# powturbo/Turbo-Range-Coder

Measured on AMD Instinct MI355X. Metric: encode+decode MB/s, order-0 static-CDF rANS, 100 MB bytes, higher is better.
Workload: dtype u32; 1 GPU; text100m: 100000000 B/GPU, static-CDF rANS, 2 states (anscdf4senc/anscdf4sdec per chunk), tables in LDS, chunk 512 B, 1 lane = 1 chunk, 64 chunks/wave; codec=anscdf4s, chunk=512, bytes_per_gpu=100000000, compressed_bytes_per_gpu=64522350, steps_in_flight=1, exchange=none

## Files before the change

include/trc_hip.h:

```cpp
#ifndef TRC_HIP_H_
#define TRC_HIP_H_
#include <stddef.h>
#include <stdint.h>

#ifdef __cplusplus
extern "C" {
#endif

enum trc_codec {
    TRC_ANS4S = 1,
    TRC_RCS1  = 2,
    TRC_RCS2  = 3,
    TRC_RCA   = 4,
    TRC_ANSA  = 5,
    TRC_RCB   = 6,
    TRC_RCAI  = 7,
    TRC_RCA4  = 8,
    TRC_RCAI4 = 9,
    TRC_ANSA4 = 10,
    TRC_RCSM  = 11,
    TRC_ANSO1 = 12,
    TRC_ANSB  = 13,
    TRC_VLCU16 = 14,  TRC_VLCU32 = 15,
    TRC_VLCV16 = 16,  TRC_VLCV32 = 17,
// ... 289 lines not shown
                               uint8_t *filters_out, trc_planes_advice *advice );
size_t trc_planes_advise_batch_work_bytes(const trc_planes_item *items, size_t count, unsigned esize, uint32_t chunk);
int    trc_planes_advise_batch_dev(unsigned filters, const trc_planes_item *items, size_t count, unsigned esize, uint32_t chunk,
                                   uint8_t *filters_out, trc_planes_advice *advice,
                                   void *d_work, size_t work_bytes, void *stream);

#define TRC_PLANES_BATCH_MAGIC 0x42435254u
typedef struct trc_planes_batch_hdr {
    uint32_t magic;
    uint8_t  version;
    uint8_t  esize;
    uint16_t zero;
    uint32_t chunk;
    uint32_t zero2;
    uint64_t count;
    uint64_t inner;
    uint64_t size;
    uint64_t bytes;
} trc_planes_batch_hdr;
typedef struct trc_planes_batch_layout {
    uint64_t inner;
    uint64_t off[8];
    uint64_t size;
} trc_planes_batch_layout;
enum { TRC_ITEMS_HOST = 0, TRC_ITEMS_DEV = 1 };
uint32_t trc_planes_batch_auto_chunk(int codec, const trc_planes_item *items, size_t count, unsigned esize);
size_t trc_planes_batch_bound(int codec, const trc_planes_item *items, size_t count, unsigned esize, uint32_t chunk, unsigned cdfnum);
int    trc_planes_batch_layout_host(int codec, const trc_planes_item *items, size_t count, unsigned esize, uint32_t chunk,
                                    unsigned cdfnum, const uint64_t *total, trc_planes_batch_layout *L);
int    trc_planes_batch_check(const void *buf, size_t buflen, size_t count_expected);
int    trc_planes_batch_info(const void *buf, size_t buflen, trc_planes_batch_hdr *h, uint64_t *n, uint8_t *filters, size_t cap);
int trc_planes_batch_pack_dev(int codec, const trc_planes_item *items, const uint8_t *filters, size_t count,
                              unsigned esize, uint32_t chunk, const uint16_t *d_cdf, unsigned cdfnum,
                              const int32_t *d_status, const uint32_t *d_clen, const void *d_payload,
                              const uint64_t *d_total, void *d_out, size_t out_bytes, uint64_t *d_size, void *stream);
int trc_decode_planes_batch_packed_dev(int codec, const void *d_cont, size_t cont_bytes,
                                       const trc_planes_item *items, const uint8_t *filters, size_t count, size_t first_item, size_t item_count,
                                       unsigned esize, uint32_t chunk, unsigned cdfnum, const uint64_t *total ,
                                       void *d_work, size_t work_bytes, void *stream);
size_t trc_encode_planes_batch_host(int codec, const trc_planes_item *items, const uint8_t *filters ,
                                    size_t count, unsigned esize, uint32_t chunk, unsigned cdfnum, int items_on,
                                    void *out, size_t outcap);
size_t trc_encode_aplanes_batch_host(int codec, const trc_planes_item *items, size_t count, unsigned esize, uint32_t chunk,
                                     unsigned cdfnum, int items_on, void *out, size_t outcap, uint8_t *filters_out );
size_t trc_decode_planes_batch_host(const void *in, size_t inlen, const trc_planes_item *items, size_t count,
                                    size_t first_item, size_t item_count, int items_on);

int trc_timing_enable(int on);
int trc_timing_pause(int paused);
int trc_timing_read(int decode, double *total_ms, int *launches);

const char *trc_kernel_name(int codec, int decode);

#ifdef __cplusplus
}
#endif
#endif
```

turbo-range-coder_amd/csrc/trc_api.hip:

```cpp
#include <hip/hip_runtime.h>
#include <mutex>
#include <stdarg.h>
#include <stdio.h>
#include <stdlib.h>
#include <string.h>

#include "../../include/trc_hip.h"
#include "trc_launch.h"

typedef unsigned short cdf_t;
static const unsigned TRC_PROB_ONE_HOST = 32768u;

static thread_local char g_err[512];
static int fail(int code, const char *fmt, ...)
{
    va_list ap; va_start(ap, fmt);
    vsnprintf(g_err, sizeof g_err, fmt, ap);
    va_end(ap);
    fprintf(stderr, "turborc_hip: ERROR: %s\n", g_err);
    return code;
}
int trc_fail(int code, const char *fmt, ...)
{
    va_list ap; va_start(ap, fmt);
// ... 117 lines not shown
#undef NONE
static constexpr int TRC_NCODECS = (int)(sizeof g_codecs / sizeof g_codecs[0]);
static constexpr bool rows_in_id_order()
{
    for (int i = 0; i < TRC_NCODECS; i++) if (g_codecs[i].id != i) return false;
    return true;
}
static_assert(rows_in_id_order(), "g_codecs[i] must be the row of id i");
static const TrcCodec &codec_row(int codec) { return g_codecs[codec > 0 && codec < TRC_NCODECS ? codec : 0]; }
static bool codec_ok(int codec) { return codec_row(codec).enc != nullptr; }
static bool ss_prm_ok(unsigned v) { return !(v & ~0x0f0fu) && (v & 0x0fu) && (v & 0x0f00u); }

static uint32_t g_chunk = 0;
static bool chunk_ok(uint32_t c) { return c >= TRC_CHUNK_MIN && c <= TRC_CHUNK_MAX && (c % 64u) == 0; }
extern "C" uint32_t trc_auto_chunk_codec(int codec, size_t n)
{
    static const uint32_t ladder[] = { 16384u, 12288u, 8192u, 6144u, 4096u, 3072u, 2048u, 1536u, 1024u, 768u, 512u };
    const TrcCodec &r = codec_row(codec);
    const double link_ns = 0.35 * (double)n / 50.0;
    const double budget_ns = link_ns > 1.7e6 ? link_ns : 1.7e6;
    const uint32_t lo = r.floor ? r.floor : TRC_CHUNK_AUTO_MIN;
    for (uint32_t c : ladder)
        if (c <= r.auto_max && (c <= lo || (double)r.wave_ns * c <= budget_ns)) return c;
    return lo;
}
extern "C" uint32_t trc_auto_chunk(size_t n) { return trc_auto_chunk_codec(TRC_ANS4S, n); }
#define TRC_ROUND_CHUNK_MAX 16384u
extern "C" uint32_t trc_round_chunk(int codec, size_t n)
{
    const TrcCodec &r = codec_row(codec);
    if (r.floor) return r.floor;
    const size_t rc = r.round_lanes;
    const size_t cap = r.chunk_max < TRC_ROUND_CHUNK_MAX ? r.chunk_max : TRC_ROUND_CHUNK_MAX;
    for (size_t k = 1;; k++) {
        size_t c = (n + rc * k - 1) / (rc * k);
        c = (c + 63u) & ~(size_t)63u;
        if (c <= cap) return c < TRC_CHUNK_AUTO_MIN ? TRC_CHUNK_AUTO_MIN : (uint32_t)c;
    }
}
extern "C" uint32_t trc_get_chunk(void)
{
    if (!g_chunk) {
        const char *e = getenv("TRC_CHUNK");
        uint32_t c = e ? (uint32_t)strtoul(e, 0, 10) : 0;
        g_chunk = chunk_ok(c) ? c : ~0u;
    }
    return g_chunk == ~0u ? 0u : g_chunk;
}
extern "C" int trc_set_chunk(uint32_t chunk)
{
    if (chunk == 0) { g_chunk = ~0u; return TRC_OK; }
    if (!chunk_ok(chunk)) return fail(TRC_E_ARG, "chunk %u: must be 0 (automatic) or a multiple of 64 in [%u,%u]", chunk, TRC_CHUNK_MIN, TRC_CHUNK_MAX);
    g_chunk = chunk;
    return TRC_OK;
}

#define TRC_INKERNEL_SCAN_MAX 8192u
static inline size_t up256(size_t x) { return (x + 255) & ~(size_t)255; }
static inline size_t scratch2_bytes(const TrcCodec &r, size_t nchunks, uint32_t chunk)
{
    const size_t rows = r.s2_lanes ? ((nchunks + 63) & ~(size_t)63) : nchunks;
    return up256(rows * ((size_t)r.s2_mul * chunk + r.s2_add) + 256);
}
static inline size_t model_area_bytes(const TrcCodec &r, size_t nchunks) { return r.model_area ? up256(r.model_area(r, nchunks)) : 0; }

extern "C" size_t trc_work_bytes(int codec, size_t n, uint32_t chunk)
{
    if (!codec) return 4096;
    const TrcCodec &r = codec_row(codec);
    if (!r.enc || !chunk_ok(chunk)) return 0;
    const size_t nchunks = (n + chunk - 1) / chunk, ngroups = (nchunks + 63) / 64;
    return up256(TRC_TAB_BYTES) + up256(4 * ngroups) + up256(8 * (ngroups + 1)) +
           up256(nchunks * ((size_t)chunk + r.pad)) + scratch2_bytes(r, nchunks, chunk) + model_area_bytes(r, nchunks) +
           (r.aux ? up256(nchunks * 8) : 0) + 4096;
}

static int carve(const TrcCodec &r, size_t n, uint32_t chunk, void *d_work, size_t work_bytes, TrcWork &w)
{
    const size_t need = trc_work_bytes(r.id, n, chunk);
    if (!need || work_bytes < need) return fail(TRC_E_WORK, "workspace %zu B < required %zu B", work_bytes, need);
    if (((uintptr_t)d_work) & 255) return fail(TRC_E_ARG, "workspace must be 256-byte aligned");
    const size_t nchunks = (n + chunk - 1) / chunk, ngroups = (nchunks + 63) / 64;
    uint8_t *p = (uint8_t *)d_work;
    w.tables = p;               p += up256(TRC_TAB_BYTES);
    w.gsum = (uint32_t *)p;     p += up256(4 * ngroups);
    static const uint32_t scan_max = getenv("TRC_SCAN_MAX") ? (uint32_t)atoi(getenv("TRC_SCAN_MAX")) : TRC_INKERNEL_SCAN_MAX;
    w.goff_area = (uint64_t *)p;
    w.goff = ngroups > scan_max ? (uint64_t *)p : nullptr;     p += up256(8 * (ngroups + 1));
    w.scratch = p;
    w.stride = chunk + r.pad;
    w.stride2 = r.s2_mul * chunk + r.s2_add;
    w.scratch2 = p + up256(nchunks * (size_t)w.stride);
    w.model = w.scratch2 + scratch2_bytes(r, nchunks, chunk);
    w.aux = (uint32_t *)(w.model + model_area_bytes(r, nchunks));
    w.nchunks = (uint32_t)nchunks; w.ngroups = (uint32_t)ngroups;
    return TRC_OK;
}

static int check_common(int codec, size_t n, uint32_t chunk, const uint16_t *d_cdf, unsigned cdfnum)
{
    const TrcCodec &r = codec_row(codec);
    if (!r.enc) return fail(TRC_E_ARG, "codec %d not available", codec);
    if (!chunk_ok(chunk)) return fail(TRC_E_ARG, "chunk %u: must be a multiple of 64 in [%u,%u]", chunk, TRC_CHUNK_MIN, TRC_CHUNK_MAX);
    if ((n + chunk - 1) / chunk > 0x7fffffffu) return fail(TRC_E_ARG, "too many chunks");
    if (chunk > r.chunk_max) return fail(TRC_E_ARG, "codec %d: chunk %u exceeds %u", r.id, chunk, r.chunk_max);
    if (r.cdf && (!d_cdf || cdfnum < 1 || cdfnum > 256)) return fail(TRC_E_CDF, "static coder needs a CDF with 1..256 symbols");
// ... 493 lines not shown
```

turbo-range-coder_amd/csrc/trc_dev.h:

```cpp
#pragma once
#include <hip/hip_runtime.h>
#include <stdint.h>

typedef uint8_t  u8;
typedef uint16_t u16;
typedef uint32_t u32;
typedef uint64_t u64;

#define TRC_WAVE        64
#define TRC_PROB_BITS   15u
#define TRC_PROB_ONE    (1u << TRC_PROB_BITS)
#define TRC_ANS_LOW     (1u << 15)

typedef u32 u32_a1 __attribute__((aligned(1)));
typedef u32 u32_a2 __attribute__((aligned(2)));
struct __attribute__((packed, aligned(2))) trc_u128_a2 { u32 x, y, z, w; };

__device__ __forceinline__ uint4 trc_ld16_a2(const u8 *p)
{
    trc_u128_a2 v = *(const trc_u128_a2 *)p;
    return make_uint4(v.x, v.y, v.z, v.w);
}
__device__ __forceinline__ u32 trc_ld32_a2(const u8 *p) { return *(const u32_a2 *)p; }

// ... 138 lines not shown
        for (u32 i = lane; i < len; i += 64) dst[i] = src[i];
        return;
    }
    u32 head = (u32)((16u - ((uintptr_t)dst & 15u)) & 15u);
    if (head > len) head = len;
    if (lane < head) dst[lane] = src[lane];
    const u32 nvec = (len - head) >> 4;
    u8 *d = dst + head; const u8 *s = src + head;
    for (u32 i = lane; i < nvec; i += 64)
        *(uint4 *)(d + (size_t)i * 16) = trc_ld16_a2(s + (size_t)i * 16);
    const u32 done = head + (nvec << 4);
    if (lane < len - done) dst[done + lane] = src[done + lane];
}

__device__ __forceinline__ void trc_wave_copy_raw(u64 rawmask, u64 off, u32 len, u8 *out_wave, u32 chunk, const u8 *payload)
{
    const u32 lane = trc_lane(), grp = lane >> 4, gl = lane & 15u;
    if (((uintptr_t)out_wave | chunk) & 15u) {
        while (rawmask) {
            const int k = __ffsll((long long)rawmask) - 1;
            rawmask &= rawmask - 1;
            const u32 olo = (u32)__shfl((int)(u32)off, k, 64), ohi = (u32)__shfl((int)(u32)(off >> 32), k, 64);
            const u32 l = (u32)__shfl((int)len, k, 64);
            trc_wave_copy(out_wave + (u64)(u32)k * chunk, payload + (((u64)ohi << 32) | olo), l);
        }
        return;
    }
    while (rawmask) {
        int mine = -1;
#pragma unroll
        for (u32 g = 0; g < 4; g++) {
            const int k = rawmask ? __ffsll((long long)rawmask) - 1 : -1;
            if (rawmask) rawmask &= rawmask - 1;
            if (g == grp) mine = k;
        }
        const int src_lane = mine < 0 ? 0 : mine;
        const u32 olo = (u32)__shfl((int)(u32)off, src_lane, 64), ohi = (u32)__shfl((int)(u32)(off >> 32), src_lane, 64);
        const u32 l = (u32)__shfl((int)len, src_lane, 64);
        if (mine >= 0) {
            u8 *d = out_wave + (u64)(u32)mine * chunk;
            const u8 *sp = payload + (((u64)ohi << 32) | olo);
            const u32 nvec = l >> 4;
            for (u32 i = gl; i < nvec; i += 16) *(uint4 *)(d + (size_t)i * 16) = trc_ld16_a2(sp + (size_t)i * 16);
            const u32 done = nvec << 4;
            if (gl < l - done) d[done + gl] = sp[done + gl];
        }
    }
}

__device__ __forceinline__ u64 trc_group_base(const u64 *goff, const u32 *gsum, u32 g)
{
    if (goff) return goff[g];
    u64 acc = 0;
    u32 i = trc_lane();
    for (; i + 448u < g; i += 512u) {
        const u32 a0 = gsum[i], a1 = gsum[i + 64], a2 = gsum[i + 128], a3 = gsum[i + 192];
        const u32 a4 = gsum[i + 256], a5 = gsum[i + 320], a6 = gsum[i + 384], a7 = gsum[i + 448];
        acc += (u64)a0 + a1 + a2 + a3 + ((u64)a4 + a5 + a6 + a7);
    }
    for (; i < g; i += 64) acc += gsum[i];
    u32 lo = (u32)acc, hi = (u32)(acc >> 32);
#pragma unroll
    for (int d = 32; d >= 1; d >>= 1) {
        const u32 l2 = (u32)__shfl_xor((int)lo, d, 64), h2 = (u32)__shfl_xor((int)hi, d, 64);
        const u64 t = ((((u64)hi) << 32) | lo) + ((((u64)h2) << 32) | l2);
        lo = (u32)t; hi = (u32)(t >> 32);
    }
    return (((u64)hi) << 32) | lo;
}

__device__ __forceinline__ float trc_u2f(u32 v)
{
    float r;
    asm("v_cvt_f32_u32_e32 %0, %1" : "=v"(r) : "v"(v));
    return r;
}

__device__ __forceinline__ u32 trc_rans_step(u32 st, u32 f, u32 g, u32 c0)
{
    const u32 q = (u32)((float)st * __builtin_amdgcn_rcpf((float)f));
    const int rm = (int)(st - __umul24(q, f));
    const u32 qe = q + (u32)(rm >> 31) + (rm >= (int)f ? 1u : 0u);
    return st + __umul24(qe, g) + c0;
}
```

turbo-range-coder_amd/csrc/trc_dir.hip:

```cpp
#include <stdlib.h>
#include "trc_dev.h"
#include "trc_launch.h"

__global__ __launch_bounds__(256) void trc_static_prep_kernel(const u16 *__restrict__ cdf, u32 cdfnum,
                                                              u8 *__restrict__ tables)
{
    __shared__ u32 c[258];
    const u32 tid = threadIdx.x;
    for (u32 i = tid; i < 258; i += 256) c[i] = (i <= cdfnum) ? (u32)cdf[i] : TRC_PROB_ONE;
    __syncthreads();
    const u32 slot = blockIdx.x * 256 + tid;
    u32 x = 0, hi = 256;
    while (x + 1 < hi) { u32 mid = (x + hi) >> 1; if (c[mid] > slot) hi = mid; else x = mid; }
    tables[TRC_TAB_LUT + slot] = (u8)x;
    if (blockIdx.x == 0) {
        const u32 c0 = c[tid], f = c[tid + 1] - c0;
        uint4 e; u32 d;
        if (f == 0) {
            e = make_uint4(0u, 0u, 0xffffffffu, 0u); d = 1u << 16;
        } else if (f == 1) {
            e = make_uint4(0xffffffffu, TRC_PROB_ONE - 1u, 1u << 16, c0 + TRC_PROB_ONE - 1u); d = (1u << 16) | c0;
        } else {
            const u32 l = 32u - (u32)__clz((int)(f - 1));
            const u32 m = (u32)((((u64)1) << (31 + l)) / f) + 1u;
// ... 43 lines not shown
        for (u32 k = 0; k < wid; k++) wbase += wsum[k];
        const u64 base = base_s;
        if (i < ngroups) goff[i] = base + wbase + inc - v;
        __syncthreads();
        if (tid == 1023) base_s = base + wbase + inc;
        __syncthreads();
    }
    if (tid == 0) { goff[ngroups] = base_s; if (total) *total = base_s; }
}
void trc_launch_scan_groups(const uint32_t *gsum, uint32_t ngroups, uint64_t *goff, uint64_t *d_total, hipStream_t s)
{
    TRC_LAUNCH_TIMED(trc_scan_groups_kernel, dim3(1), dim3(1024), 0, s, gsum, ngroups, goff, d_total);
}

__global__ __launch_bounds__(256) void trc_range_dir_kernel(const u32 *__restrict__ clen, u32 nchunks, u64 n, u32 chunk,
                                                            const u64 *__restrict__ goff_full, u32 first, u32 count,
                                                            u32 *__restrict__ gsum_sub, u64 *__restrict__ goff_sub)
{
    const u32 ngroups_sub = (count + 63u) >> 6, end = first + count;
    const u32 j = blockIdx.x * 4u + (threadIdx.x >> 6), lane = trc_lane();
    if (j > ngroups_sub) return;
    const u32 b = trc_min(first + 64u * j, end);
    auto clamped = [&](u32 c) -> u32 {
        const u64 left = n - (u64)c * chunk;
        return trc_min(clen[c], left < chunk ? (u32)left : chunk);
    };
    const u32 below = (b & ~63u) + lane, mine = b + lane;
    const u32 pre = trc_wave_sum(below < b ? clamped(below) : 0u);
    const u32 sum = trc_wave_sum(mine < end ? clamped(mine) : 0u);
    if (lane == 0) {
        goff_sub[j] = goff_full[b >> 6] + pre;
        if (j < ngroups_sub) gsum_sub[j] = sum;
    }
}
void trc_launch_range_dir(const uint32_t *d_clen, uint32_t nchunks, size_t n, uint32_t chunk, const uint64_t *goff_full,
                          uint32_t first, uint32_t count, uint32_t *gsum_sub, uint64_t *goff_sub, hipStream_t s)
{
    const uint32_t waves = (count + 63u) / 64u + 1u;
    hipLaunchKernelGGL(trc_range_dir_kernel, dim3((waves + 3u) / 4u), dim3(256), 0, s, d_clen, nchunks, (u64)n, chunk, goff_full,
                       first, count, gsum_sub, goff_sub);
}

#ifndef TRC_GATHER_VPT
#define TRC_GATHER_VPT 6
#endif
#ifndef TRC_GATHER_ATTR
#define TRC_GATHER_ATTR
#endif
template <int PARTS>
__global__ __launch_bounds__(256) TRC_GATHER_ATTR void trc_gather_kernel(const u8 *__restrict__ in, u64 n, u32 chunk, u32 nchunks,
                                                         const u8 *__restrict__ scratch, u32 stride, int from_end,
                                                         const u8 *__restrict__ scratch2, u32 stride2, const u32 *__restrict__ aux,
                                                         const u32 *__restrict__ clen, const u64 *__restrict__ goff,
                                                         const u32 *__restrict__ gsum, u32 ngroups,
                                                         u8 *__restrict__ payload, u64 *__restrict__ total, u64 *__restrict__ goff_out)
{
    constexpr u32 NP = 64u * PARTS;
    constexpr u32 TPP = 256u / NP;
    constexpr u32 VPT = TRC_GATHER_VPT;
    __shared__ u32 ex_s[NP + 1];
    __shared__ u64 src_s[NP];
    __shared__ u64 base_s;
    const u32 g = blockIdx.x, tid = threadIdx.x, lane = tid & 63u, wid = tid >> 6;
    if (wid == 1 || blockDim.x == 64) {
        const u64 b = trc_group_base(goff, gsum, g);
        if (lane == 0) { base_s = b; if (goff_out) goff_out[g] = b; }
    }
    if (wid == 0) {
        const u32 c = g * 64 + lane;
        const u32 l = c < nchunks ? clen[c] : 0u;
        const u64 cstart = (u64)c * chunk;
        const u32 len = c < nchunks ? (u32)((n - cstart) < chunk ? (n - cstart) : chunk) : 0u;
        const bool raw = l == len;
        const u32 inc = trc_wave_incl_scan(l);
        if (PARTS == 1) {
            ex_s[lane] = inc - l;
            src_s[lane] = (u64)(uintptr_t)(raw ? in + cstart : from_end ? scratch + (u64)(c + 1) * stride - l : scratch + (u64)c * stride);
        } else {
            const u8 *a = scratch + (u64)c * stride;
            const u32 la = (raw || c >= nchunks) ? l : from_end >= 3 ? aux[2 * c] : 4u + *(const u32 *)a;
            ex_s[2 * lane] = inc - l; ex_s[2 * lane + 1] = inc - l + la;
            src_s[2 * lane] = (u64)(uintptr_t)(raw ? in + cstart : from_end == 4 ? scratch + (u64)(c + 1) * stride - la : a);
            src_s[2 * lane + 1] = (u64)(uintptr_t)(from_end == 3 ? scratch + (u64)(c + 1) * stride - (l - la) :
                                                   from_end == 4 ? scratch2 + (u64)(c + 1) * stride2 - (l - la) : scratch2 + (u64)c * stride2);
        }
        if (lane == 63) ex_s[NP] = inc;
    }
    __syncthreads();
    const u64 base = base_s;
    const u32 tot = ex_s[NP];
    if (total && g == ngroups - 1 && tid == 0) *total = base + tot;
    u8 *dst0 = payload + base;
    auto src_of = [&](u32 p) -> const u8 * { return (const u8 *)(uintptr_t)src_s[p]; };

    u32 head = (u32)((16u - ((uintptr_t)dst0 & 15u)) & 15u);
    if (head > tot) head = tot;
    const u32 nvec = (tot - head) >> 4;
    const u32 tail0 = head + (nvec << 4);
    for (u32 b = tid; b < head + (tot - tail0); b += 256) {
        const u32 d = b < head ? b : tail0 + (b - head);
        u32 lo = 0, hi = NP;
        while (lo + 1 < hi) { const u32 mid = (lo + hi) >> 1; if (ex_s[mid] <= d) lo = mid; else hi = mid; }
        dst0[d] = src_of(lo)[d - ex_s[lo]];
    }
    {
        const u32 k = tid / TPP, sub = tid % TPP;
        const u32 e0 = ex_s[k], e1 = ex_s[k + 1];
        const u32 v_lo = e0 <= head ? 0u : (e0 - head + 15u) >> 4;
        u32 v_hi = e1 <= head ? 0u : (e1 - head + 15u) >> 4;
        if (v_hi > nvec) v_hi = nvec;
        const u8 *sa = src_of(k);
        const u8 *sb = k + 1 < NP ? src_of(k + 1) : sa;
        const u32 e2 = ex_s[k + 2 > NP ? NP : k + 2];
        const u32 pl = e1 - e0;
        const bool a16 = pl >= 16u;
        const bool b16 = k + 1 < NP && e2 - e1 >= 16u;
        auto bytewise = [&](u32 dv) {
            u32 kk = k;
            const u8 *p = sa;
            for (u32 q = 0; q < 16; q++) {
                while (dv + q >= ex_s[kk + 1]) { kk++; p = src_of(kk); }
                dst0[dv + q] = p[dv + q - ex_s[kk]];
            }
        };
        if (!a16) {
            if (sub == 0 && v_lo < v_hi) bytewise(head + (v_lo << 4));
            return;
        }
        for (u32 v0 = v_lo + sub; v0 < v_hi; v0 += VPT * TPP) {
            uint4 a[VPT], b[VPT];
            u32 d[VPT];
            bool ok[VPT];
#pragma unroll
            for (int j = 0; j < (int)VPT; j++) {
                const u32 v = v0 + TPP * (u32)j;
                ok[j] = v < v_hi;
                d[j] = head + ((ok[j] ? v : v0) << 4);
                a[j] = make_uint4(0u, 0u, 0u, 0u);
                if (ok[j]) a[j] = trc_ld16_a2_global(sa + trc_min(d[j] - e0, pl - 16u));
                b[j] = a[j];
            }
#pragma unroll
            for (int j = 0; j < (int)VPT; j++)
                if (ok[j] && d[j] + 16u > e1 && b16) b[j] = trc_ld16_a2_global(sb);
#pragma unroll
            for (int j = 0; j < (int)VPT; j++) {
                if (!ok[j]) continue;
                const u32 sp = e1 - d[j];
                if (sp >= 16u) { *(uint4 *)(dst0 + d[j]) = a[j]; continue; }
                if (b16) *(uint4 *)(dst0 + d[j]) = trc_splice16(a[j], b[j], 16u - sp);
                else bytewise(d[j]);
            }
        }
    }
}
void trc_launch_gather(const uint8_t *d_in, size_t n, uint32_t chunk, const TrcWork &w, TrcGather mode,
                       const uint32_t *d_clen, uint8_t *d_payload, uint64_t *d_total, hipStream_t s)
{
    const int from_end = mode;
    if (from_end >= 2)
        TRC_LAUNCH_TIMED((trc_gather_kernel<2>), dim3(w.ngroups), dim3(256), 0, s, d_in, (u64)n, chunk, w.nchunks,
                           w.scratch, w.stride, from_end >= 3 ? from_end : 0, w.scratch2, w.stride2, w.aux, d_clen, w.goff, w.gsum, w.ngroups,
                           d_payload, w.goff ? (u64 *)nullptr : d_total, w.goff ? (u64 *)nullptr : w.goff_area);
    else
        TRC_LAUNCH_TIMED((trc_gather_kernel<1>), dim3(w.ngroups), dim3(256), 0, s, d_in, (u64)n, chunk, w.nchunks,
                           w.scratch, w.stride, from_end, w.scratch2, w.stride2, w.aux, d_clen, w.goff, w.gsum, w.ngroups,
                           d_payload, w.goff ? (u64 *)nullptr : d_total, w.goff ? (u64 *)nullptr : w.goff_area);
}

#define TRC_HIST2_WAVE_LDS (128u * 16u * 4u)
#define TRC_HIST2_WAVES 16u
#define TRC_HIST2_ROUND_VECS 1023u
__global__ __launch_bounds__(1024) void trc_hist2_kernel(const u8 *__restrict__ in, u64 n, u64 *__restrict__ hist, u32 round_vecs)
{
    extern __shared__ __attribute__((aligned(16))) u8 smem[];
    typedef __attribute__((address_space(3))) u32 lds_u32;
    const u32 tid = threadIdx.x, lane = tid & 63u, wv = tid >> 6;
    u32 *mine = (u32 *)(smem + wv * TRC_HIST2_WAVE_LDS);
    u64 *tot = (u64 *)(smem + TRC_HIST2_WAVES * TRC_HIST2_WAVE_LDS);
    const u32 col = trc_lds_addr(mine) + (lane & 15u) * 4u;
    if (tid < 256u) tot[tid] = 0;
    const u64 nvec = n >> 4, stride = (u64)gridDim.x * 1024;
    const uint4 *v = (const uint4 *)in;
    auto count = [&](u32 w) __attribute__((always_inline)) {
#pragma unroll
        for (int k = 0; k < 4; k++) {
            const u32 a = (__builtin_amdgcn_ubfe(w, 8 * k + 1, 7) << 6) + col;
            const u32 inc = __umul24(__builtin_amdgcn_ubfe(w, 8 * k, 1), 0xffffu) + 1u;
            __hip_atomic_fetch_add((lds_u32 *)(uintptr_t)a, inc, __ATOMIC_RELAXED, __HIP_MEMORY_SCOPE_WAVEFRONT);
        }
    };
    auto count4 = [&](const uint4 q) __attribute__((always_inline)) { count(q.x); count(q.y); count(q.z); count(q.w); };
    for (u64 r0 = 0; r0 == 0 || r0 < nvec; r0 += stride * round_vecs) {
        for (u32 r = lane; r < 128u * 16u; r += 64u) mine[r] = 0;
        u64 i = r0 + (u64)blockIdx.x * 1024 + tid;
        u32 left = round_vecs;
        if (left >= 2u && i + stride < nvec) {
            uint4 q0 = v[i], q1 = v[i + stride];
            left -= 2u; i += 2 * stride;
            for (; left >= 2u && i + stride < nvec; left -= 2u, i += 2 * stride) {
                const uint4 n0 = v[i], n1 = v[i + stride];
                count4(q0); count4(q1);
                q0 = n0; q1 = n1;
            }
            count4(q0); count4(q1);
        }
        for (; left && i < nvec; left--, i += stride) count4(v[i]);
        if (r0 == 0 && blockIdx.x == 0 && wv == 0)
            for (u64 t = (nvec << 4) + lane; t < n; t += 64) {
                const u32 b = in[t];
                __hip_atomic_fetch_add((lds_u32 *)(uintptr_t)(col + (b >> 1) * 64u), (b & 1u) ? 0x10000u : 1u, __ATOMIC_RELAXED, __HIP_MEMORY_SCOPE_WAVEFRONT);
            }
        u32 lo0 = 0, hi0 = 0, lo1 = 0, hi1 = 0;
#pragma unroll
        for (u32 c4 = 0; c4 < 4u; c4++) {
            const uint4 a = *(const uint4 *)(mine + lane * 16u + c4 * 4u), b = *(const uint4 *)(mine + (lane + 64u) * 16u + c4 * 4u);
            lo0 += (a.x & 0xffffu) + (a.y & 0xffffu) + (a.z & 0xffffu) + (a.w & 0xffffu); hi0 += (a.x >> 16) + (a.y >> 16) + (a.z >> 16) + (a.w >> 16);
            lo1 += (b.x & 0xffffu) + (b.y & 0xffffu) + (b.z & 0xffffu) + (b.w & 0xffffu); hi1 += (b.x >> 16) + (b.y >> 16) + (b.z >> 16) + (b.w >> 16);
        }
// ... 60 lines not shown
```

turbo-range-coder_amd/csrc/trc_launch.h:

```cpp
#pragma once
#include <hip/hip_runtime.h>
#include <hip/hip_ext.h>
#include <stddef.h>
#include <stdint.h>
#include <stdlib.h>

bool trc_tm_next(hipEvent_t *start, hipEvent_t *stop);
#define TRC_LAUNCH_TIMED(kern, grid, block, lds, stream, ...)                                                      \
    do {                                                                                                         \
        hipEvent_t tm_a_, tm_b_;                                                                                 \
        if (trc_tm_next(&tm_a_, &tm_b_)) hipExtLaunchKernelGGL(kern, grid, block, (uint32_t)(lds), stream, tm_a_, tm_b_, 0, __VA_ARGS__); \
        else hipLaunchKernelGGL(kern, grid, block, lds, stream, __VA_ARGS__);                                    \
    } while (0)

bool trc_first_use_on_device(unsigned long long *mask);
#define TRC_RAISE_LDS_ONCE(kern, bytes)                                                                            \
    do {                                                                                                         \
        static unsigned long long seen_ = 0;                                                                     \
        if (trc_first_use_on_device(&seen_))                                                                     \
            (void)hipFuncSetAttribute((const void *)kern, hipFuncAttributeMaxDynamicSharedMemorySize, (int)(bytes)); \
    } while (0)

#define TRC_LDS_ONE_PER_CU (82u * 1024u)
static inline bool trc_nib_big(uint32_t ngroups)
{
    static const int env = getenv("TRC_NIB_BIG") ? atoi(getenv("TRC_NIB_BIG")) : -1;
    return env >= 0 ? env != 0 : (ngroups >= 2048u && ngroups <= 12u * 256u);
}

struct TrcGate { const uint32_t *flag; uint32_t part; };
extern thread_local TrcGate trc_gate_tls;
struct TrcProg { uint32_t *counters; uint32_t *host_flags; uint32_t part; };
extern thread_local TrcProg trc_prog_tls;
bool trc_prog_ok(int codec);
bool trc_gate_ok(int codec);

struct TrcWork {
    uint8_t  *tables;
    uint32_t *gsum;
    uint64_t *goff;
    uint64_t *goff_area;
    uint8_t  *scratch;
    uint32_t  stride;
    uint8_t  *scratch2;
    uint32_t  stride2;
    uint32_t  nchunks, ngroups;
    uint8_t  *model;
    uint32_t *aux;
    uint32_t  ss_prm;
};
#define TRC_O1_MODEL_BYTES (256u * 17u * 32u)

#define TRC_TAB_ENC   0
#define TRC_TAB_DEC   4096
#define TRC_TAB_LUT   8192
#define TRC_TAB_CDF   40960
#define TRC_TAB_BYTES 45056

void trc_launch_static_prep(const uint16_t *d_cdf, unsigned cdfnum, uint8_t *tables, hipStream_t s);

enum TrcGather {
    TRC_GATHER_START = 0,
    TRC_GATHER_END = 1,
    TRC_GATHER_TWO = 2,
    TRC_GATHER_AUX = 3,
    TRC_GATHER_VLA = 4,
};

void trc_launch_group_sums(const uint32_t *d_clen, uint32_t nchunks, size_t n, uint32_t chunk, uint32_t *gsum, hipStream_t s);
void trc_launch_scan_groups(const uint32_t *gsum, uint32_t ngroups, uint64_t *goff, uint64_t *d_total, hipStream_t s);
void trc_launch_range_dir(const uint32_t *d_clen, uint32_t nchunks, size_t n, uint32_t chunk, const uint64_t *goff_full,
                          uint32_t first, uint32_t count, uint32_t *gsum_sub, uint64_t *goff_sub, hipStream_t s);
void trc_launch_gather(const uint8_t *d_in, size_t n, uint32_t chunk, const TrcWork &w, TrcGather mode,
                       const uint32_t *d_clen, uint8_t *d_payload, uint64_t *d_total, hipStream_t s);

struct TrcCodec;
typedef void TrcEncFn(const TrcCodec &c, const uint8_t *d_in, size_t n, uint32_t chunk, const TrcWork &w, uint32_t *d_clen, hipStream_t s);
typedef void TrcDecFn(const TrcCodec &c, const uint8_t *d_payload, const uint32_t *d_clen, size_t n, uint32_t chunk,
                      const TrcWork &w, uint8_t *d_out, hipStream_t s);

struct TrcCodec {
    int id;
    TrcEncFn *enc;
    TrcDecFn *dec;
    int8_t k;
    int8_t streams;
    int8_t nibble;
    bool low4;
    int8_t variant;
    int8_t zz;
    int8_t elem;
    TrcGather gather;
    bool cdf;
    bool ss;
    bool aux;
    bool gate;
    bool prog;
    uint16_t wave_ns;
    uint32_t round_lanes;
    uint32_t auto_max;
    uint32_t floor;
    uint32_t chunk_max;
    uint16_t pad;
    uint8_t s2_mul;
    uint16_t s2_add;
    bool s2_lanes;
    size_t (*model_area)(const TrcCodec &c, size_t nchunks);
    size_t (*slice_model)(const TrcCodec &c);
    const char *kernel_enc, *kernel_dec;
};

TrcEncFn trc_launch_ans4s_enc;  TrcDecFn trc_launch_ans4s_dec;
TrcEncFn trc_launch_rcs_enc;    TrcDecFn trc_launch_rcs_dec;
TrcEncFn trc_launch_rcb_enc;    TrcDecFn trc_launch_rcb_dec;
TrcEncFn trc_launch_o1bit_enc;  TrcDecFn trc_launch_o1bit_dec;
TrcEncFn trc_launch_int_enc;    TrcDecFn trc_launch_int_dec;
size_t trc_int_model_bytes(int k, size_t ngroups);
TrcEncFn trc_launch_bvlc_enc;   TrcDecFn trc_launch_bvlc_dec;
size_t trc_bvlc_model_bytes(int k, size_t nchunks);
TrcEncFn trc_launch_word_enc;   TrcDecFn trc_launch_word_dec;
size_t trc_word_model_bytes(int k);
size_t trc_word_slots(int k, size_t nchunks);
TrcEncFn trc_launch_nibbit_enc; TrcDecFn trc_launch_nibbit_dec;
TrcEncFn trc_launch_ssbit_enc;  TrcDecFn trc_launch_ssbit_dec;
void trc_o1bit_fill(uint8_t *model, size_t bytes, hipStream_t s);
TrcEncFn trc_launch_rca_enc;    TrcDecFn trc_launch_rca_dec;
TrcEncFn trc_launch_rcv_enc;    TrcDecFn trc_launch_rcv_dec;
// ... 13 lines not shown
```

turbo-range-coder_amd/trc.py:

```python
import ctypes as C
import os
import subprocess

import numpy as np

PKG = os.path.dirname(os.path.abspath(__file__))
ROOT = os.path.dirname(PKG)
LIB = os.environ.get("TRC_LIB") or os.path.join(PKG, "libturborc_hip.so")

ANS4S, RCS1, RCS2, RCA, ANSA, RCB, RCAI, RCA4, RCAI4, ANSA4, RCSM, ANSO1, ANSB = 1, 2, 3, 4, 5, 6, 7, 8, 9, 10, 11, 12, 13
VLCU16, VLCU32, VLCV16, VLCV32, VLCVZ16, VLCVZ32 = 14, 15, 16, 17, 18, 19
VLAU16, VLAUZ16, VLAV16, VLAVZ16, VLAV32, VLAVZ32 = 20, 21, 22, 23, 24, 25
RCV8, RCVI8 = 26, 27
RCC1, RCX1 = 28, 29
RCG8, RCG16, RCG32, RCGZ8, RCGZ16, RCGZ32 = 30, 31, 32, 33, 34, 35
RCR8, RCR16, RCR32, RCRZ8, RCRZ16, RCRZ32 = 36, 37, 38, 39, 40, 41
INTBIT = ((RCG8, 1), (RCG16, 2), (RCG32, 4), (RCGZ8, 1), (RCGZ16, 2), (RCGZ32, 4),
          (RCR8, 1), (RCR16, 2), (RCR32, 4), (RCRZ8, 1), (RCRZ16, 2), (RCRZ32, 4))
RCBV16, RCBV32, RCBVZ16, RCBVZ32, RCBVG16, RCBVG32, RCBVGZ16, RCBVGZ32 = 43, 44, 45, 46, 47, 48, 49, 50
BVLC = ((RCBV16, 2), (RCBV32, 4), (RCBVZ16, 2), (RCBVZ32, 4),
        (RCBVG16, 2), (RCBVG32, 4), (RCBVGZ16, 2), (RCBVGZ32, 4))
RCW16, RCW32, RCCW32, RCC2W32 = 52, 53, 54, 55
WORD = ((RCW16, 2), (RCW32, 4), (RCCW32, 4), (RCC2W32, 4))
RC4, RC4C, RCU3 = 58, 59, 60
# ... 165 lines not shown
        l.trc_encode_planes_batch_dev.restype = C.c_int
        l.trc_encode_planes_batch_dev.argtypes = [C.c_int, _it, _sz, C.c_uint, C.c_uint32, _vp, C.c_uint, _vp, _vp, _vp, _vp, _vp, _sz, _vp]
        l.trc_decode_planes_batch_dev.restype = C.c_int
        l.trc_decode_planes_batch_dev.argtypes = [C.c_int, _vp, _vp, _it, _sz, _sz, _sz, C.c_uint, C.c_uint32, _vp, C.c_uint, _vp, _sz, _vp]
        _fl = C.POINTER(C.c_uint8)
        l.trc_planes_split_fbatch_dev.restype = C.c_int
        l.trc_planes_split_fbatch_dev.argtypes = [_it, _fl] + l.trc_planes_split_batch_dev.argtypes[1:]
        l.trc_planes_join_fbatch_dev.restype = C.c_int
        l.trc_planes_join_fbatch_dev.argtypes = [_vp, _sz, _it, _fl] + l.trc_planes_join_batch_dev.argtypes[3:]
        l.trc_encode_fplanes_batch_dev.restype = C.c_int
        l.trc_encode_fplanes_batch_dev.argtypes = [C.c_int, _it, _fl] + l.trc_encode_planes_batch_dev.argtypes[2:]
        l.trc_decode_fplanes_batch_dev.restype = C.c_int
        l.trc_decode_fplanes_batch_dev.argtypes = [C.c_int, _vp, _vp, _it, _fl] + l.trc_decode_planes_batch_dev.argtypes[4:]
        _ad = C.POINTER(PlanesAdvice)
        l.trc_planes_hist_batch_bytes.restype = _sz; l.trc_planes_hist_batch_bytes.argtypes = [_sz, C.c_uint]
        l.trc_planes_hist_batch_dev.restype = C.c_int
        l.trc_planes_hist_batch_dev.argtypes = [C.c_uint, _it, _sz, _sz, _sz, C.c_uint, C.c_uint32, _vp, _vp, _sz, _vp]
        l.trc_planes_advise_batch.restype = C.c_int
        l.trc_planes_advise_batch.argtypes = [_vp, C.c_uint, C.c_uint, _it, _sz, _fl, _ad]
        l.trc_planes_advise_batch_work_bytes.restype = _sz; l.trc_planes_advise_batch_work_bytes.argtypes = [_it, _sz, C.c_uint, C.c_uint32]
        l.trc_planes_advise_batch_dev.restype = C.c_int
        l.trc_planes_advise_batch_dev.argtypes = [C.c_uint, _it, _sz, C.c_uint, C.c_uint32, _fl, _ad, _vp, _sz, _vp]
        l.trc_planes_batch_auto_chunk.restype = C.c_uint32; l.trc_planes_batch_auto_chunk.argtypes = [C.c_int, _it, _sz, C.c_uint]
        l.trc_planes_batch_bound.restype = _sz; l.trc_planes_batch_bound.argtypes = [C.c_int, _it, _sz, C.c_uint, C.c_uint32, C.c_uint]
        l.trc_planes_batch_layout_host.restype = C.c_int
        l.trc_planes_batch_layout_host.argtypes = [C.c_int, _it, _sz, C.c_uint, C.c_uint32, C.c_uint, C.POINTER(C.c_uint64), C.POINTER(PlanesBatchLayout)]
        l.trc_planes_batch_check.restype = C.c_int; l.trc_planes_batch_check.argtypes = [_vp, _sz, _sz]
        l.trc_planes_batch_info.restype = C.c_int
        l.trc_planes_batch_info.argtypes = [_vp, _sz, C.POINTER(PlanesBatchHdr), C.POINTER(C.c_uint64), _fl, _sz]
        l.trc_planes_batch_pack_dev.restype = C.c_int
        l.trc_planes_batch_pack_dev.argtypes = [C.c_int, _it, _fl, _sz, C.c_uint, C.c_uint32, _vp, C.c_uint, _vp, _vp, _vp, _vp, _vp, _sz, _vp, _vp]
        l.trc_decode_planes_batch_packed_dev.restype = C.c_int
        l.trc_decode_planes_batch_packed_dev.argtypes = [C.c_int, _vp, _sz, _it, _fl, _sz, _sz, _sz, C.c_uint, C.c_uint32, C.c_uint,
                                                         C.POINTER(C.c_uint64), _vp, _sz, _vp]
        l.trc_encode_planes_batch_host.restype = _sz
        l.trc_encode_planes_batch_host.argtypes = [C.c_int, _it, _fl, _sz, C.c_uint, C.c_uint32, C.c_uint, C.c_int, _vp, _sz]
        l.trc_encode_aplanes_batch_host.restype = _sz
        l.trc_encode_aplanes_batch_host.argtypes = [C.c_int, _it, _sz, C.c_uint, C.c_uint32, C.c_uint, C.c_int, _vp, _sz, _fl]
        l.trc_decode_planes_batch_host.restype = _sz
        l.trc_decode_planes_batch_host.argtypes = [_vp, _sz, _it, _sz, _sz, _sz, C.c_int]
        l.trc_encode_host.restype = _sz; l.trc_encode_host.argtypes = [C.c_int, _vp, _sz, C.c_uint32, _vp, _sz, _vp, C.c_uint]
        l.trc_decode_host.restype = _sz; l.trc_decode_host.argtypes = [C.c_int, _vp, _sz, _vp, _sz, _vp, C.c_uint]
        l.trc_container_bound.restype = _sz; l.trc_container_bound.argtypes = [_sz, C.c_uint32]
        l.trc_container_check.restype = C.c_int; l.trc_container_check.argtypes = [_vp, _sz, C.c_int, _sz]
        l.trc_host_plan.restype = C.c_int
        l.trc_host_plan.argtypes = [C.c_int, _sz, C.c_uint32, C.c_int, C.c_int, C.POINTER(_sz), C.c_int, C.POINTER(C.c_uint32)]
        l.trc_host_pin.restype = C.c_int; l.trc_host_pin.argtypes = [_vp, _sz]
        l.trc_host_unpin.restype = C.c_int; l.trc_host_unpin.argtypes = [_vp]
        l.trc_timing_enable.restype = C.c_int; l.trc_timing_enable.argtypes = [C.c_int]
        l.trc_timing_pause.restype = C.c_int; l.trc_timing_pause.argtypes = [C.c_int]
        l.trc_timing_read.restype = C.c_int
        l.trc_timing_read.argtypes = [C.c_int, C.POINTER(C.c_double), C.POINTER(C.c_int)]
        l.trc_kernel_name.restype = C.c_char_p; l.trc_kernel_name.argtypes = [C.c_int, C.c_int]
        l.trc_set_devices.restype = C.c_int; l.trc_set_devices.argtypes = [C.POINTER(C.c_int), C.c_int]
        l.trc_get_devices.restype = C.c_int; l.trc_get_devices.argtypes = [C.POINTER(C.c_int), C.c_int]
        _lib = l
    return _lib


class TrcError(RuntimeError):
    pass


def _chk(rc):
    if rc != 0:
        raise TrcError("libturborc_hip rc=%d: %s" % (rc, lib().trc_last_error().decode()))


def timing_enable(on=True):
    _chk(lib().trc_timing_enable(1 if on else 0))


def timing_pause(paused=True):
    _chk(lib().trc_timing_pause(1 if paused else 0))


def timing_read(decode):
    ms, cnt = C.c_double(0), C.c_int(0)
    _chk(lib().trc_timing_read(2 if decode == 2 else 1 if decode else 0, C.byref(ms), C.byref(cnt)))
    return ms.value, cnt.value


def ss_prm(prm):
    return int(prm[0]) | int(prm[1]) << 8


def _cdfnum(codec, cdfnum, prm):
    return cdfnum if codec in STATIC else ss_prm(prm) if codec in SSBIT else 0


def nchunks(n, chunk):
    return (n + chunk - 1) // chunk


def range_work_bytes(codec, n, chunk, count):
    return lib().trc_range_work_bytes(codec, n, chunk, count)


class DeviceCoder:

    def __init__(self, codec, n, chunk=4096, device="cuda"):
        import torch
        self.torch = torch
        self.codec, self.n, self.chunk = codec, n, chunk
        self.nch = nchunks(n, chunk)
        self.dev = torch.device(device)
        u8 = torch.uint8
        self.work_bytes = lib().trc_work_bytes(codec, n, chunk)
        if self.work_bytes == 0:
            raise TrcError("bad (codec, n, chunk)")
        self.work = torch.empty(self.work_bytes + PAD, dtype=u8, device=self.dev)
        self.clen = torch.zeros(max(self.nch, 1) + 64, dtype=torch.int32, device=self.dev)
        self.payload = torch.zeros(n + PAD + 64, dtype=u8, device=self.dev)
        self.total = torch.zeros(2, dtype=torch.int64, device=self.dev)
        self.cdf = torch.zeros(264, dtype=torch.int16, device=self.dev)
        self.status = torch.zeros(4, dtype=torch.int32, device=self.dev)
        self.cdfnum = 0
        self.tables_ready = 0
        self.range_work, self.range_work_bytes = None, 0
        self.range_tables = 0

    def _stream(self):
        return self.torch.cuda.current_stream(self.dev).cuda_stream

    def _tables(self):
        if self.codec in STATIC:
            _chk(lib().trc_tables_dev(self.cdf.data_ptr(), self.cdfnum, self.work.data_ptr(), self.work_bytes, self._stream()))
            self.tables_ready = TABLES_READY
            self.range_tables = 0

    def set_cdf(self, cdf_np, cdfnum):
        t = self.torch.from_numpy(np.ascontiguousarray(cdf_np[:cdfnum + 1]).view(np.int16))
        self.cdf[:cdfnum + 1].copy_(t)
# ... 785 lines not shown
```

Before: 737,700 MB/s.

## Make gather kernel persistent with occupancy-sized grid and per-workgroup chunk ranges

The gather kernel now launches a grid sized to device occupancy (CUs times resident blocks) instead of one workgroup per 64-chunk group. Each workgroup takes a contiguous chunk range and loops over 64-chunk tiles, carrying a running output base and adding a prefix over the partial leading group. The group-base reduction also reads gsum as uint4 vectors. This cuts launch and per-block setup overhead, at the cost of serial tile iterations with extra barriers inside each workgroup and less parallelism per tile.

```diff
diff --git a/include/trc_hip.h b/include/trc_hip.h
--- a/include/trc_hip.h
+++ b/include/trc_hip.h
@@ -365,6 +365,9 @@
 
 const char *trc_kernel_name(int codec, int decode);
 
+int trc_gather_wgs(int wgs);
+int trc_gather_range(uint32_t nchunks, uint32_t wgs, uint32_t w, uint32_t *first, uint32_t *count);
+
 #ifdef __cplusplus
 }
 #endif
diff --git a/turbo-range-coder_amd/csrc/trc_api.hip b/turbo-range-coder_amd/csrc/trc_api.hip
--- a/turbo-range-coder_amd/csrc/trc_api.hip
+++ b/turbo-range-coder_amd/csrc/trc_api.hip
@@ -193,6 +193,19 @@
     if (chunk == 0) { g_chunk = ~0u; return TRC_OK; }
     if (!chunk_ok(chunk)) return fail(TRC_E_ARG, "chunk %u: must be 0 (automatic) or a multiple of 64 in [%u,%u]", chunk, TRC_CHUNK_MIN, TRC_CHUNK_MAX);
     g_chunk = chunk;
+    return TRC_OK;
+}
+
+extern "C" int trc_gather_wgs(int wgs)
+{
+    if (wgs < 0) return fail(TRC_E_ARG, "gather workgroups %d: must be 0 (automatic) or positive", wgs);
+    trc_gather_wgs_forced = wgs;
+    return TRC_OK;
+}
+extern "C" int trc_gather_range(uint32_t nchunks, uint32_t wgs, uint32_t w, uint32_t *first, uint32_t *count)
+{
+    if (!wgs || w >= wgs || !first || !count) return fail(TRC_E_ARG, "gather range: workgroup %u of %u", w, wgs);
+    trc_gather_plan(nchunks, wgs, w, first, count);
     return TRC_OK;
 }
 
diff --git a/turbo-range-coder_amd/csrc/trc_dev.h b/turbo-range-coder_amd/csrc/trc_dev.h
--- a/turbo-range-coder_amd/csrc/trc_dev.h
+++ b/turbo-range-coder_amd/csrc/trc_dev.h
@@ -214,13 +214,16 @@
 {
     if (goff) return goff[g];
     u64 acc = 0;
+    const uint4 *q = (const uint4 *)gsum;
+    const u32 nq = g >> 2;
     u32 i = trc_lane();
-    for (; i + 448u < g; i += 512u) {
-        const u32 a0 = gsum[i], a1 = gsum[i + 64], a2 = gsum[i + 128], a3 = gsum[i + 192];
-        const u32 a4 = gsum[i + 256], a5 = gsum[i + 320], a6 = gsum[i + 384], a7 = gsum[i + 448];
-        acc += (u64)a0 + a1 + a2 + a3 + ((u64)a4 + a5 + a6 + a7);
-    }
-    for (; i < g; i += 64) acc += gsum[i];
+    for (; i + 192u < nq; i += 256u) {
+        const uint4 a0 = q[i], a1 = q[i + 64], a2 = q[i + 128], a3 = q[i + 192];
+        acc += ((u64)a0.x + a0.y + a0.z + a0.w) + ((u64)a1.x + a1.y + a1.z + a1.w) +
+               (((u64)a2.x + a2.y + a2.z + a2.w) + ((u64)a3.x + a3.y + a3.z + a3.w));
+    }
+    for (; i < nq; i += 64) { const uint4 a = q[i]; acc += (u64)a.x + a.y + a.z + a.w; }
+    if ((nq << 2) + trc_lane() < g) acc += gsum[(nq << 2) + trc_lane()];
     u32 lo = (u32)acc, hi = (u32)(acc >> 32);
 #pragma unroll
     for (int d = 32; d >= 1; d >>= 1) {
diff --git a/turbo-range-coder_amd/csrc/trc_dir.hip b/turbo-range-coder_amd/csrc/trc_dir.hip
--- a/turbo-range-coder_amd/csrc/trc_dir.hip
+++ b/turbo-range-coder_amd/csrc/trc_dir.hip
@@ -119,7 +119,7 @@
                                                          const u8 *__restrict__ scratch, u32 stride, int from_end,
                                                          const u8 *__restrict__ scratch2, u32 stride2, const u32 *__restrict__ aux,
                                                          const u32 *__restrict__ clen, const u64 *__restrict__ goff,
-                                                         const u32 *__restrict__ gsum, u32 ngroups,
+                                                         const u32 *__restrict__ gsum,
                                                          u8 *__restrict__ payload, u64 *__restrict__ total, u64 *__restrict__ goff_out)
 {
     constexpr u32 NP = 64u * PARTS;
@@ -128,16 +128,18 @@
     __shared__ u32 ex_s[NP + 1];
     __shared__ u64 src_s[NP];
     __shared__ u64 base_s;
-    const u32 g = blockIdx.x, tid = threadIdx.x, lane = tid & 63u, wid = tid >> 6;
-    if (wid == 1 || blockDim.x == 64) {
-        const u64 b = trc_group_base(goff, gsum, g);
-        if (lane == 0) { base_s = b; if (goff_out) goff_out[g] = b; }
-    }
-    if (wid == 0) {
-        const u32 c = g * 64 + lane;
-        const u32 l = c < nchunks ? clen[c] : 0u;
+    __shared__ u32 pre_s;
+    const u32 tid = threadIdx.x, lane = tid & 63u, wid = tid >> 6;
+    u32 first, count;
+    trc_gather_plan(nchunks, gridDim.x, blockIdx.x, &first, &count);
+    if (count == 0) return;
+    const u32 end = first + count;
+    auto dir_fill = [&](u32 c0, u32 tn) {
+        const u32 c = c0 + lane;
+        const bool valid = lane < tn;
+        const u32 l = valid ? clen[c] : 0u;
         const u64 cstart = (u64)c * chunk;
-        const u32 len = c < nchunks ? (u32)((n - cstart) < chunk ? (n - cstart) : chunk) : 0u;
+        const u32 len = valid ? (u32)((n - cstart) < chunk ? (n - cstart) : chunk) : 0u;
         const bool raw = l == len;
         const u32 inc = trc_wave_incl_scan(l);
         if (PARTS == 1) {
@@ -145,93 +147,137 @@
             src_s[lane] = (u64)(uintptr_t)(raw ? in + cstart : from_end ? scratch + (u64)(c + 1) * stride - l : scratch + (u64)c * stride);
         } else {
             const u8 *a = scratch + (u64)c * stride;
-            const u32 la = (raw || c >= nchunks) ? l : from_end >= 3 ? aux[2 * c] : 4u + *(const u32 *)a;
+            const u32 la = (raw || !valid) ? l : from_end >= 3 ? aux[2 * c] : 4u + *(const u32 *)a;
             ex_s[2 * lane] = inc - l; ex_s[2 * lane + 1] = inc - l + la;
             src_s[2 * lane] = (u64)(uintptr_t)(raw ? in + cstart : from_end == 4 ? scratch + (u64)(c + 1) * stride - la : a);
             src_s[2 * lane + 1] = (u64)(uintptr_t)(from_end == 3 ? scratch + (u64)(c + 1) * stride - (l - la) :
                                                    from_end == 4 ? scratch2 + (u64)(c + 1) * stride2 - (l - la) : scratch2 + (u64)c * stride2);
         }
         if (lane == 63) ex_s[NP] = inc;
-    }
-    __syncthreads();
-    const u64 base = base_s;
-    const u32 tot = ex_s[NP];
-    if (total && g == ngroups - 1 && tid == 0) *total = base + tot;
-    u8 *dst0 = payload + base;
+    };
+    if (wid == 1) {
+        const u64 b = trc_group_base(goff, gsum, first >> 6);
+        if (lane == 0) base_s = b;
+    }
+    if (wid == 2) {
+        const u32 below = (first & ~63u) + lane;
+        const u32 pre = trc_wave_sum(below < first ? clen[below] : 0u);
+        if (lane == 0) pre_s = pre;
+    }
+    if (wid == 0) dir_fill(first, trc_min(64u, count));
+    __syncthreads();
+    u64 base = base_s + pre_s;
     auto src_of = [&](u32 p) -> const u8 * { return (const u8 *)(uintptr_t)src_s[p]; };
-
-    u32 head = (u32)((16u - ((uintptr_t)dst0 & 15u)) & 15u);
-    if (head > tot) head = tot;
-    const u32 nvec = (tot - head) >> 4;
-    const u32 tail0 = head + (nvec << 4);
-    for (u32 b = tid; b < head + (tot - tail0); b += 256) {
-        const u32 d = b < head ? b : tail0 + (b - head);
-        u32 lo = 0, hi = NP;
-        while (lo + 1 < hi) { const u32 mid = (lo + hi) >> 1; if (ex_s[mid] <= d) lo = mid; else hi = mid; }
-        dst0[d] = src_of(lo)[d - ex_s[lo]];
-    }
-    {
-        const u32 k = tid / TPP, sub = tid % TPP;
-        const u32 e0 = ex_s[k], e1 = ex_s[k + 1];
-        const u32 v_lo = e0 <= head ? 0u : (e0 - head + 15u) >> 4;
-        u32 v_hi = e1 <= head ? 0u : (e1 - head + 15u) >> 4;
-        if (v_hi > nvec) v_hi = nvec;
-        const u8 *sa = src_of(k);
-        const u8 *sb = k + 1 < NP ? src_of(k + 1) : sa;
-        const u32 e2 = ex_s[k + 2 > NP ? NP : k + 2];
-        const u32 pl = e1 - e0;
-        const bool a16 = pl >= 16u;
-        const bool b16 = k + 1 < NP && e2 - e1 >= 16u;
-        auto bytewise = [&](u32 dv) {
-            u32 kk = k;
-            const u8 *p = sa;
-            for (u32 q = 0; q < 16; q++) {
-                while (dv + q >= ex_s[kk + 1]) { kk++; p = src_of(kk); }
-                dst0[dv + q] = p[dv + q - ex_s[kk]];
+    for (u32 c0 = first; c0 < end; c0 += 64u) {
+        const u32 tn = trc_min(64u, end - c0);
+        if (c0 != first) {
+            __syncthreads();
+            if (wid == 0) dir_fill(c0, tn);
+            __syncthreads();
+        }
+        const u32 tot = ex_s[NP];
+        if (tid == 0) {
+            const u32 cg = (c0 + 63u) & ~63u;
+            if (goff_out && cg < c0 + tn) goff_out[cg >> 6] = base + ex_s[(cg - c0) * PARTS];
+            if (total && c0 + tn == nchunks) *total = base + tot;
+        }
+        u8 *dst0 = payload + base;
+
+        u32 head = (u32)((16u - ((uintptr_t)dst0 & 15u)) & 15u);
+        if (head > tot) head = tot;
+        const u32 nvec = (tot - head) >> 4;
+        const u32 tail0 = head + (nvec << 4);
+        for (u32 b = tid; b < head + (tot - tail0); b += 256) {
+            const u32 d = b < head ? b : tail0 + (b - head);
+            u32 lo = 0, hi = NP;
+            while (lo + 1 < hi) { const u32 mid = (lo + hi) >> 1; if (ex_s[mid] <= d) lo = mid; else hi = mid; }
+            dst0[d] = src_of(lo)[d - ex_s[lo]];
+        }
+        {
+            const u32 k = tid / TPP, sub = tid % TPP;
+            const u32 e0 = ex_s[k], e1 = ex_s[k + 1];
+            const u32 v_lo = e0 <= head ? 0u : (e0 - head + 15u) >> 4;
+            u32 v_hi = e1 <= head ? 0u : (e1 - head + 15u) >> 4;
+            if (v_hi > nvec) v_hi = nvec;
+            const u8 *sa = src_of(k);
+            const u8 *sb = k + 1 < NP ? src_of(k + 1) : sa;
+            const u32 e2 = ex_s[k + 2 > NP ? NP : k + 2];
+            const u32 pl = e1 - e0;
+            const bool a16 = pl >= 16u;
+            const bool b16 = k + 1 < NP && e2 - e1 >= 16u;
+            auto bytewise = [&](u32 dv) {
+                u32 kk = k;
+                const u8 *p = sa;
+                for (u32 q = 0; q < 16; q++) {
+                    while (dv + q >= ex_s[kk + 1]) { kk++; p = src_of(kk); }
+                    dst0[dv + q] = p[dv + q - ex_s[kk]];
+                }
+            };
+            if (!a16) {
+                if (sub == 0 && v_lo < v_hi) bytewise(head + (v_lo << 4));
+            } else {
+                for (u32 v0 = v_lo + sub; v0 < v_hi; v0 += VPT * TPP) {
+                    uint4 a[VPT], b[VPT];
+                    u32 d[VPT];
+                    bool ok[VPT];
+#pragma unroll
+                    for (int j = 0; j < (int)VPT; j++) {
+                        const u32 v = v0 + TPP * (u32)j;
+                        ok[j] = v < v_hi;
+                        d[j] = head + ((ok[j] ? v : v0) << 4);
+                        a[j] = make_uint4(0u, 0u, 0u, 0u);
+                        if (ok[j]) a[j] = trc_ld16_a2_global(sa + trc_min(d[j] - e0, pl - 16u));
+                        b[j] = a[j];
+                    }
+#pragma unroll
+                    for (int j = 0; j < (int)VPT; j++)
+                        if (ok[j] && d[j] + 16u > e1 && b16) b[j] = trc_ld16_a2_global(sb);
+#pragma unroll
+                    for (int j = 0; j < (int)VPT; j++) {
+                        if (!ok[j]) continue;
+                        const u32 sp = e1 - d[j];
+                        if (sp >= 16u) { *(uint4 *)(dst0 + d[j]) = a[j]; continue; }
+                        if (b16) *(uint4 *)(dst0 + d[j]) = trc_splice16(a[j], b[j], 16u - sp);
+                        else bytewise(d[j]);
+                    }
+                }
             }
-        };
-        if (!a16) {
-            if (sub == 0 && v_lo < v_hi) bytewise(head + (v_lo << 4));
-            return;
-        }
-        for (u32 v0 = v_lo + sub; v0 < v_hi; v0 += VPT * TPP) {
-            uint4 a[VPT], b[VPT];
-            u32 d[VPT];
-            bool ok[VPT];
-#pragma unroll
-            for (int j = 0; j < (int)VPT; j++) {
-                const u32 v = v0 + TPP * (u32)j;
-                ok[j] = v < v_hi;
-                d[j] = head + ((ok[j] ? v : v0) << 4);
-                a[j] = make_uint4(0u, 0u, 0u, 0u);
-                if (ok[j]) a[j] = trc_ld16_a2_global(sa + trc_min(d[j] - e0, pl - 16u));
-                b[j] = a[j];
-            }
-#pragma unroll
-            for (int j = 0; j < (int)VPT; j++)
-                if (ok[j] && d[j] + 16u > e1 && b16) b[j] = trc_ld16_a2_global(sb);
-#pragma unroll
-            for (int j = 0; j < (int)VPT; j++) {
-                if (!ok[j]) continue;
-                const u32 sp = e1 - d[j];
-                if (sp >= 16u) { *(uint4 *)(dst0 + d[j]) = a[j]; continue; }
-                if (b16) *(uint4 *)(dst0 + d[j]) = trc_splice16(a[j], b[j], 16u - sp);
-                else bytewise(d[j]);
-            }
-        }
-    }
-}
+        }
+        base += tot;
+    }
+}
+
+template <int PARTS>
+static uint32_t trc_gather_wgs_auto(uint32_t ngroups)
+{
+    static uint32_t held[64];
+    int dev = 0;
+    (void)hipGetDevice(&dev);
+    dev = dev >= 0 && dev < 64 ? dev : 0;
+    if (!held[dev]) {
+        int per_cu = 0, cus = 0;
+        if (hipOccupancyMaxActiveBlocksPerMultiprocessor(&per_cu, trc_gather_kernel<PARTS>, 256, 0) != hipSuccess || per_cu < 1) per_cu = 4;
+        if (hipDeviceGetAttribute(&cus, hipDeviceAttributeMultiprocessorCount, dev) != hipSuccess || cus < 1) cus = 256;
+        held[dev] = (uint32_t)per_cu * (uint32_t)cus;
+    }
+    return held[dev] < ngroups ? held[dev] : ngroups;
+}
+int trc_gather_wgs_forced = 0;
 void trc_launch_gather(const uint8_t *d_in, size_t n, uint32_t chunk, const TrcWork &w, TrcGather mode,
                        const uint32_t *d_clen, uint8_t *d_payload, uint64_t *d_total, hipStream_t s)
 {
     const int from_end = mode;
+    const char *env = getenv("TRC_GATHER_WGS");
+    const int forced = trc_gather_wgs_forced > 0 ? trc_gather_wgs_forced : env ? atoi(env) : 0;
+    const uint32_t wgs = forced > 0 ? (uint32_t)(forced < (1 << 22) ? forced : (1 << 22)) :
+                         from_end >= 2 ? trc_gather_wgs_auto<2>(w.ngroups) : trc_gather_wgs_auto<1>(w.ngroups);
     if (from_end >= 2)
-        TRC_LAUNCH_TIMED((trc_gather_kernel<2>), dim3(w.ngroups), dim3(256), 0, s, d_in, (u64)n, chunk, w.nchunks,
-                           w.scratch, w.stride, from_end >= 3 ? from_end : 0, w.scratch2, w.stride2, w.aux, d_clen, w.goff, w.gsum, w.ngroups,
+        TRC_LAUNCH_TIMED((trc_gather_kernel<2>), dim3(wgs), dim3(256), 0, s, d_in, (u64)n, chunk, w.nchunks,
+                           w.scratch, w.stride, from_end >= 3 ? from_end : 0, w.scratch2, w.stride2, w.aux, d_clen, w.goff, w.gsum,
                            d_payload, w.goff ? (u64 *)nullptr : d_total, w.goff ? (u64 *)nullptr : w.goff_area);
     else
-        TRC_LAUNCH_TIMED((trc_gather_kernel<1>), dim3(w.ngroups), dim3(256), 0, s, d_in, (u64)n, chunk, w.nchunks,
-                           w.scratch, w.stride, from_end, w.scratch2, w.stride2, w.aux, d_clen, w.goff, w.gsum, w.ngroups,
+        TRC_LAUNCH_TIMED((trc_gather_kernel<1>), dim3(wgs), dim3(256), 0, s, d_in, (u64)n, chunk, w.nchunks,
+                           w.scratch, w.stride, from_end, w.scratch2, w.stride2, w.aux, d_clen, w.goff, w.gsum,
                            d_payload, w.goff ? (u64 *)nullptr : d_total, w.goff ? (u64 *)nullptr : w.goff_area);
 }
 
diff --git a/turbo-range-coder_amd/csrc/trc_launch.h b/turbo-range-coder_amd/csrc/trc_launch.h
--- a/turbo-range-coder_amd/csrc/trc_launch.h
+++ b/turbo-range-coder_amd/csrc/trc_launch.h
@@ -73,6 +73,15 @@
                           uint32_t first, uint32_t count, uint32_t *gsum_sub, uint64_t *goff_sub, hipStream_t s);
 void trc_launch_gather(const uint8_t *d_in, size_t n, uint32_t chunk, const TrcWork &w, TrcGather mode,
                        const uint32_t *d_clen, uint8_t *d_payload, uint64_t *d_total, hipStream_t s);
+__host__ __device__ inline void trc_gather_plan(uint32_t nchunks, uint32_t wgs, uint32_t w, uint32_t *first, uint32_t *count)
+{
+    const uint32_t q = nchunks / wgs, r = nchunks - q * wgs;
+    const uint64_t ar = (uint64_t)w * r, br = ar + r;
+    const uint32_t a = w * q + (br >> 32 ? (uint32_t)(ar / wgs) : (uint32_t)ar / wgs);
+    const uint32_t b = (w + 1u) * q + (br >> 32 ? (uint32_t)(br / wgs) : (uint32_t)br / wgs);
+    *first = a; *count = b - a;
+}
+extern int trc_gather_wgs_forced;
 
 struct TrcCodec;
 typedef void TrcEncFn(const TrcCodec &c, const uint8_t *d_in, size_t n, uint32_t chunk, const TrcWork &w, uint32_t *d_clen, hipStream_t s);
diff --git a/turbo-range-coder_amd/trc.py b/turbo-range-coder_amd/trc.py
--- a/turbo-range-coder_amd/trc.py
+++ b/turbo-range-coder_amd/trc.py
@@ -241,6 +241,9 @@
         l.trc_timing_read.restype = C.c_int
         l.trc_timing_read.argtypes = [C.c_int, C.POINTER(C.c_double), C.POINTER(C.c_int)]
         l.trc_kernel_name.restype = C.c_char_p; l.trc_kernel_name.argtypes = [C.c_int, C.c_int]
+        l.trc_gather_wgs.restype = C.c_int; l.trc_gather_wgs.argtypes = [C.c_int]
+        l.trc_gather_range.restype = C.c_int
+        l.trc_gather_range.argtypes = [C.c_uint32, C.c_uint32, C.c_uint32, C.POINTER(C.c_uint32), C.POINTER(C.c_uint32)]
         l.trc_set_devices.restype = C.c_int; l.trc_set_devices.argtypes = [C.POINTER(C.c_int), C.c_int]
         l.trc_get_devices.restype = C.c_int; l.trc_get_devices.argtypes = [C.POINTER(C.c_int), C.c_int]
         _lib = l
@@ -268,6 +271,16 @@
     ms, cnt = C.c_double(0), C.c_int(0)
     _chk(lib().trc_timing_read(2 if decode == 2 else 1 if decode else 0, C.byref(ms), C.byref(cnt)))
     return ms.value, cnt.value
+
+
+def gather_wgs(wgs=0):
+    _chk(lib().trc_gather_wgs(wgs))
+
+
+def gather_range(nchunks, wgs, w):
+    first, count = C.c_uint32(0), C.c_uint32(0)
+    _chk(lib().trc_gather_range(nchunks, wgs, w, C.byref(first), C.byref(count)))
+    return first.value, count.value
 
 
 def ss_prm(prm):
```

Result: no change. 740,800 MB/s (median of 6 runs) (+0.4%).
